# Minimap2onGPU/mm2-gb

Hardware: AMD Instinct MI355X
Metric: chaining anchor-pairs/s (higher is better)
Workload: dtype int32+f32

## Files before the change

include/mm2gb_chain.h:

```cpp
#ifndef MM2GB_CHAIN_H
#define MM2GB_CHAIN_H

#include <stddef.h>
#include <stdint.h>

#ifdef __cplusplus
extern "C" {
#endif

#define MM2GB_VERSION "0.1-mi355x"

typedef struct { uint64_t x, y; } mm2gb_anchor_t;

typedef struct {
	int max_iter, max_dist_x, max_dist_y, max_skip, bw, min_cnt, min_score, is_cdna, n_seg;
	float chn_pen_gap, chn_pen_skip;
} mm2gb_misc_t;

typedef struct {
	int     num_streams;
	int     min_n;
	int64_t long_seg_buffer_size;
	int64_t max_total_n;
	int     max_read;
// ... 24 lines not shown
void mm2gb_config_defaults(mm2gb_config_t *cfg);
int  mm2gb_config_parse(const char *json_text, mm2gb_config_t *cfg);
int  mm2gb_config_load(const char *path, mm2gb_config_t *cfg);

int  mm2gb_device_count(void);
int  mm2gb_device_numa_node(int device);
int  mm2gb_pin_thread_to_device(int device);
int  mm2gb_numa_cpus_for_bdf(const char *bdf, const char *sysfs_root_dir, int32_t *node_out, int32_t *cpus, int32_t max_cpus);
mm2gb_engine_t *mm2gb_engine_create(const mm2gb_config_t *cfg, const mm2gb_misc_t *misc, int device);
void mm2gb_engine_destroy(mm2gb_engine_t *eng);
int  mm2gb_engine_set_misc(mm2gb_engine_t *eng, const mm2gb_misc_t *misc);
int  mm2gb_engine_set_chain_skip(mm2gb_engine_t *eng, int keep);
int  mm2gb_engine_last_score_form(const mm2gb_engine_t *eng);
int  mm2gb_engine_last_score_mode(mm2gb_engine_t *eng);
int  mm2gb_engine_band_groups(const mm2gb_engine_t *eng, int64_t *out);
int  mm2gb_engine_band_shape(const mm2gb_engine_t *eng, int *out6);
int  mm2gb_engine_skip_stats(mm2gb_engine_t *eng, int64_t *out6);
int  mm2gb_engine_device(const mm2gb_engine_t *eng);
int  mm2gb_engine_cu_count(const mm2gb_engine_t *eng);
void mm2gb_engine_gang_counts(const mm2gb_engine_t *eng, int64_t *chunks, int64_t *workgroups);
int  mm2gb_has_gang_build(void);
int  mm2gb_engine_reserve(mm2gb_engine_t *eng, int64_t n_anchors, int64_t n_reads);

int mm2gb_score_host(mm2gb_engine_t *eng, int64_t n_reads, const int64_t *offsets, const mm2gb_anchor_t *anchors,
                     int32_t *f, int32_t *p, mm2gb_stats_t *stats);
int mm2gb_score_device(mm2gb_engine_t *eng, int64_t n_reads, const int64_t *d_offsets, const mm2gb_anchor_t *d_anchors,
                       int64_t n_anchors, int32_t *d_f, int32_t *d_p);
int mm2gb_engine_sync(mm2gb_engine_t *eng);
int mm2gb_engine_stats(mm2gb_engine_t *eng, mm2gb_stats_t *stats);
void *mm2gb_engine_stream(mm2gb_engine_t *eng);
// ... 443 lines not shown
```

mm2-gb_amd/__init__.py:

```python
import ctypes as C
import os

import numpy as np

_HERE = os.path.dirname(os.path.abspath(__file__))
LIB_PATH = os.environ.get("MM2GB_LIB_PATH") or os.path.join(_HERE, "libmm2gb_chain.so")
INT32_MAX = 2**31 - 1


class Misc(C.Structure):
    _fields_ = [("max_iter", C.c_int), ("max_dist_x", C.c_int), ("max_dist_y", C.c_int), ("max_skip", C.c_int),
                ("bw", C.c_int), ("min_cnt", C.c_int), ("min_score", C.c_int), ("is_cdna", C.c_int), ("n_seg", C.c_int),
                ("chn_pen_gap", C.c_float), ("chn_pen_skip", C.c_float)]


class _RangeCfg(C.Structure):
    _fields_ = [("blockdim", C.c_int), ("cut_check_anchors", C.c_int), ("anchor_per_block", C.c_int)]


class _ScoreCfg(C.Structure):
    _fields_ = [("micro_batch", C.c_int), ("mid_blockdim", C.c_int), ("short_griddim", C.c_int), ("long_griddim", C.c_int),
                ("mid_griddim", C.c_int), ("long_seg_cutoff", C.c_int), ("mid_seg_cutoff", C.c_int)]


# ... 264 lines not shown

    def last_score_form(self):
        return int(lib().mm2gb_engine_last_score_form(self._h))

    def last_score_mode(self):
        m = int(lib().mm2gb_engine_last_score_mode(self._h))
        if m < 0:
            raise Mm2gbError(lib().mm2gb_last_error().decode())
        return m

    def band_groups(self):
        out = (C.c_int64 * 2)()
        _check(lib().mm2gb_engine_band_groups(self._h, out))
        return int(out[0]), int(out[1])

    def band_shape(self):
        L = lib()
        L.mm2gb_engine_band_shape.argtypes = [C.c_void_p, C.POINTER(C.c_int)]
        out = (C.c_int * 6)()
        _check(L.mm2gb_engine_band_shape(self._h, out))
        return dict(zip(("slab", "lag_wave", "lag_team4", "lag_team8", "lag_wg", "min_window"), (int(v) for v in out)))

    def cu_count(self):
        L = lib()
        L.mm2gb_engine_cu_count.argtypes = [C.c_void_p]
        return int(L.mm2gb_engine_cu_count(self._h))

    def skip_stats(self):
        L = lib()
        L.mm2gb_engine_skip_stats.argtypes = [C.c_void_p, C.c_void_p]
# ... 1552 lines not shown
```

mm2-gb_amd/csrc/chain_dev.h:

```cpp
#pragma once
#include <hip/hip_runtime.h>
#include <stdint.h>

namespace mm2gb {

struct DevParams {
	int   max_dist_x, max_dist_y, bw, max_iter, n_seg, is_cdna;
	int   dq_lim;
	int   lut_last;
	int   lut_base;
	int   lut_clamp;
	int   free_sweep;
	int   band_slab;
	int   band_lag_wave;
	int   band_lag_team4;
	int   band_lag_team8;
	int   band_lag_wg;
	int   band_min_window;
	float gap, skip;
};
constexpr int BAND_LAG_WAVE = 0, BAND_LAG_TEAM4 = 256, BAND_LAG_TEAM8 = 512, BAND_LAG_WG = 512;
constexpr int BAND_MIN_WINDOW = 256;

enum : unsigned { FLAG_ANY_SEGID = 1u,
                  FLAG_NO_LUT = 2u };

constexpr int LUT_LDS_TOTAL = 31 * 2560;
constexpr int LUT_ENTRIES   = 5120;
constexpr int LUT_LDS_BASE  = LUT_LDS_TOTAL - LUT_ENTRIES * 4;
constexpr int LUT_BIAS      = (1 << 30) + (1 << 16);

constexpr int PLAN_BLOCK = 1024;
#ifndef MM2GB_PLAN_THREADS
#define MM2GB_PLAN_THREADS 256
#endif
constexpr int PLAN_THREADS = MM2GB_PLAN_THREADS;
constexpr int COST_PER_ANCHOR = 16;
// ... 37 lines not shown
	int64_t  *chunk_pp;
	int32_t  *chunk_kk, *chunk_blk;
	int64_t  *tile_sums, *tile_base;
	int32_t  *bins;
	int32_t  *order;
	int32_t  *long_list;
	int32_t  *mid_list;
	int32_t  *counters;
	int64_t  *totals;
	unsigned *flags;
	const int32_t *lut;
	int64_t  *dbg;
	GangSlot *gang_slots;
};
enum { CNT_NCHUNK = 0, CNT_CURSOR = 1, CNT_NLONG = 2, CNT_LCURSOR = 3, CNT_NTRACK = 4, CNT_NCLAMP = 5, CNT_NMID = 6, CNT_MCURSOR = 7,
       CNT_NGANG = 12,
       CNT_GANG_STRIPS = 13,
       CNT_GANG_WGS = 14,
       CNT_BAND_WAVE = 16,
       CNT_BAND_TEAM = 17,
       CNT_WORDS = 18 };

struct LaunchCfg {
	int score_grid;
	int host_mode;
	int ring_slots;
	int big_team;
	int whole_wg_pct;
	int team4_all;
	int team4_share_pct;
	int gang_max;
	int gang_pct;
	int gang_pairs;
	int64_t long_min_cost;
	int     long_min_window;
	int     wide_window;
};

void launch_window(const DevBatch &b, const DevParams &P, hipStream_t s);
void launch_plan(const DevBatch &b, const LaunchCfg &cfg, hipStream_t s);
void launch_score(const DevBatch &b, const DevParams &P, const LaunchCfg &cfg, hipStream_t s);
constexpr int SKIP_STAT_WORDS = 6;
void launch_skip_fill(const DevBatch &b, const DevParams &P, int max_skip, int32_t *mark, unsigned long long *stats, int n_cu, hipStream_t s);
void launch_build_lut(int *d_lut, const DevParams &P, hipStream_t s);
size_t score_lds_bytes(const DevParams &P, int host_mode, int ring_slots);
int  score_set_lds_limit(size_t bytes);
enum { SCORE_MODE_LUT = 0, SCORE_MODE_FAST = 1, SCORE_MODE_GENERAL = 2 };

}
```

mm2-gb_amd/csrc/chain_kernels.hip:

```cpp
#include <hip/hip_runtime.h>
#include <stdint.h>
#include <limits.h>
#include <algorithm>
#include "chain_dev.h"
#include "wave_scan.h"

namespace mm2gb {

#define WAVE 64

__device__ __forceinline__ int lane_id() { return threadIdx.x & (WAVE - 1); }
__device__ __forceinline__ int bcast(int v, int src_lane) { return __builtin_amdgcn_readlane(v, src_lane); }
__device__ __forceinline__ int first_lane(int v) { return __builtin_amdgcn_readfirstlane(v); }
__device__ __forceinline__ int wave_max_i32_dpp(int v)
{
	v = max(v, __builtin_amdgcn_update_dpp(INT_MIN, v, 0x111, 0xf, 0xf, false));
	v = max(v, __builtin_amdgcn_update_dpp(INT_MIN, v, 0x112, 0xf, 0xf, false));
	v = max(v, __builtin_amdgcn_update_dpp(INT_MIN, v, 0x114, 0xf, 0xf, false));
	v = max(v, __builtin_amdgcn_update_dpp(INT_MIN, v, 0x118, 0xf, 0xf, false));
	v = max(v, __builtin_amdgcn_update_dpp(INT_MIN, v, 0x142, 0xa, 0xf, false));
	v = max(v, __builtin_amdgcn_update_dpp(INT_MIN, v, 0x143, 0xc, 0xf, false));
	return __builtin_amdgcn_readlane(v, WAVE - 1);
}
__device__ __forceinline__ int prev_lane(int v) { return __builtin_amdgcn_update_dpp(v, v, 0x138, 0xf, 0xf, false); }
__device__ __forceinline__ int a_x(const DevBatch &b, int i) { return ((const int*)b.raw)[(size_t)i * 4]; }
__device__ __forceinline__ int a_y(const DevBatch &b, int i) { return ((const int*)b.raw)[(size_t)i * 4 + 2]; }
// ... 219 lines not shown
		b.blk_firstcut[blk] = blk_cut;
		b.blk_pairs[blk] = (int64_t)my_pairs;
		b.blk_clamped[blk] = my_clamp;
	}
}

constexpr int PLANNER_THREADS = 1024;
constexpr int N_SMALL_TEAMS_PLAN = 4;
#ifndef MM2GB_COST_BINS_PER_OCTAVE
#define MM2GB_COST_BINS_PER_OCTAVE 16
#endif
constexpr int COST_SUB = MM2GB_COST_BINS_PER_OCTAVE;
constexpr int COST_SUB_LOG = COST_SUB == 16 ? 4 : COST_SUB == 8 ? 3 : 2;
constexpr int COST_BINS = 64 * COST_SUB;
static_assert(COST_BINS <= PLAN_COST_BINS, "the engine allocates PLAN_COST_BINS bins per list");
enum { LIST_WAVE = 0, LIST_BIG = 1, LIST_TEAM4 = 2, N_LISTS = 3 };

__device__ __forceinline__ int cost_bin(int64_t c)
{
	if (c <= 0) return 0;
	const int msb = 63 - __clzll(c);
	const int frac = msb >= COST_SUB_LOG ? (int)((c >> (msb - COST_SUB_LOG)) & (COST_SUB - 1)) : 0;
	return min(COST_BINS - 1, msb * COST_SUB + frac);
}

template <typename T>
__device__ T block_exclusive_scan(T v, T *s_tmp , T *total)
{
	T inc = v;
	for (int off = 1; off < WAVE; off <<= 1) {
		T o = __shfl_up(inc, off);
// ... 69 lines not shown
	for (int k = threadIdx.x; k < N_LISTS * COST_BINS; k += blockDim.x) (&s_hist[0][0])[k] = 0;
	__syncthreads();
	const int n_chunks = b.counters[CNT_NCHUNK];
	int n_track = 0;
	long long big_cost = 0;
	for (int64_t c = (int64_t)blockIdx.x * blockDim.x + threadIdx.x; c < n_chunks; c += (int64_t)gridDim.x * blockDim.x) {
		const bool last = c + 1 >= n_chunks;
		const int start = b.chunk_start[c], end = last ? (int)b.n : b.chunk_start[c + 1];
		const long long pp_next = last ? b.totals[0] : b.chunk_pp[c + 1];
		const long long kk_next = last ? b.totals[1] : (long long)b.chunk_kk[c + 1] + b.blk_clamped[b.chunk_blk[c + 1]];
		const bool track = kk_next - b.chunk_kk[c] > 0;
		const long long cost = (pp_next - b.chunk_pp[c]) + (long long)(end - start) * COST_PER_ANCHOR;
		const long long len = end - start;
		const bool heavy = cfg.ring_slots > 0 && cost >= cfg.long_min_cost && len * cfg.long_min_window <= cost;
		int list = LIST_WAVE;
		if (heavy) {
			const int blk0 = b.chunk_blk[c], blk_end = last ? (int)b.n_blocks : b.chunk_blk[c + 1];
			int wmax = b.blk_wmax[2 * blk0 + 1];
			for (int k = blk0 + 1; k < blk_end; ++k) wmax = max(wmax, b.blk_wmax[2 * k]);
			if (!last) wmax = max(wmax, b.blk_wmax[2 * blk_end]);
			const int need_slots = (wmax + WAVE - 1) / WAVE + 1;
			const int big_slots = cfg.ring_slots / (16 / cfg.big_team), small_slots = cfg.ring_slots / 4;
			const bool lut_build = cfg.host_mode == SCORE_MODE_LUT && !(b.flags[0] & (FLAG_ANY_SEGID | FLAG_NO_LUT));
			const bool small_share = lut_build && (cfg.team4_all || (cfg.team4_share_pct > 0 &&
			                         cost * 100 * cfg.score_grid * N_SMALL_TEAMS_PLAN <= (long long)cfg.team4_share_pct * b.totals[0]));
			if (len * cfg.wide_window > cost && need_slots <= small_slots) list = LIST_TEAM4;
			else if (need_slots <= big_slots) list = small_share ? LIST_TEAM4 : LIST_BIG;
		}
		b.chunk_end[c] = end;
		b.chunk_cost[c] = cost;
		b.chunk_track[c] = (uint8_t)((track ? 1 : 0) | (list << 1));
		n_track += track;
		if (list == LIST_BIG) big_cost += cost;
		atomicAdd(&s_hist[list][cost_bin(cost)], 1);
	}
	__syncthreads();
	for (int k = threadIdx.x; k < N_LISTS * COST_BINS; k += blockDim.x) {
		const int v = (&s_hist[0][0])[k];
		if (v) atomicAdd(&b.bins[k], v);
	}
	for (int off = WAVE / 2; off > 0; off >>= 1) { n_track += __shfl_xor(n_track, off); big_cost += __shfl_xor(big_cost, off); }
	if (lane_id() == 0 && n_track) atomicAdd(&b.counters[CNT_NTRACK], n_track);
	if (lane_id() == 0 && big_cost) atomicAdd((unsigned long long*)&b.totals[2], (unsigned long long)big_cost);
}

__global__ __launch_bounds__(64) void plan_bins(DevBatch b)
{
	if (threadIdx.x < N_LISTS) {
		int acc = 0;
		int *bins = b.bins + threadIdx.x * COST_BINS;
		for (int k = COST_BINS - 1; k >= 0; --k) { const int v = bins[k]; bins[k] = acc; acc += v; }
		if (threadIdx.x == LIST_BIG) b.counters[CNT_NLONG] = acc;
		if (threadIdx.x == LIST_TEAM4) b.counters[CNT_NMID] = acc;
	}
	if (threadIdx.x == 0) { b.counters[CNT_CURSOR] = 0; b.counters[CNT_LCURSOR] = 0; b.counters[CNT_MCURSOR] = 0; }
}

__global__ __launch_bounds__(256) void plan_scatter(DevBatch b)
{
	__shared__ int s_cnt[N_LISTS * COST_BINS], s_base[N_LISTS * COST_BINS];
	const int n_chunks = b.counters[CNT_NCHUNK];
	for (int64_t c0 = (int64_t)blockIdx.x * blockDim.x; c0 < n_chunks; c0 += (int64_t)gridDim.x * blockDim.x) {
		for (int k = threadIdx.x; k < N_LISTS * COST_BINS; k += blockDim.x) s_cnt[k] = 0;
		__syncthreads();
		const int64_t c = c0 + threadIdx.x;
		int key = -1, rank = 0;
		if (c < n_chunks) {
			key = ((b.chunk_track[c] >> 1) & 3) * COST_BINS + cost_bin(b.chunk_cost[c]);
			rank = atomicAdd(&s_cnt[key], 1);
		}
		__syncthreads();
		for (int k = threadIdx.x; k < N_LISTS * COST_BINS; k += blockDim.x) if (s_cnt[k]) s_base[k] = atomicAdd(&b.bins[k], s_cnt[k]);
		__syncthreads();
		if (key >= 0) {
			int *dst = key >= LIST_TEAM4 * COST_BINS ? b.mid_list : key >= LIST_BIG * COST_BINS ? b.long_list : b.order;
			dst[s_base[key] + rank] = (int)c;
		}
		__syncthreads();
	}
}

__global__ __launch_bounds__(256) void plan_gangs(DevBatch b, LaunchCfg cfg)
{
	__shared__ int s_want[256], s_pos[256], s_first[256];
	const int n_long = b.counters[CNT_NLONG];
	const int t = threadIdx.x;
	int want = 0, ci = -1;
	if (t < n_long && cfg.gang_max >= 2 && !(b.flags[0] & (FLAG_ANY_SEGID | FLAG_NO_LUT))) {
		ci = b.long_list[t];
		const long long cost = b.chunk_cost[ci], total = b.totals[0] + (long long)b.n * COST_PER_ANCHOR;
// ... 556 lines not shown
		plain_steps(tl, need & (0xffffull << (16 * q)), bestv);
		if (q < 3) on_quarter(q, bestv);
	}
}

__device__ __forceinline__ bool pair_score_uniform(const DevParams &P, int xi, int yi, int xj, int yj, int tagj, int &sc_out)
{
	const int dq = yi - yj, dr = xi - xj, span = tagj & 0xff;
	const int dg = dr < dq ? dr : dq;
	const int diff = dr - dq;
	const int dd = diff < 0 ? -diff : diff;
	sc_out = (span < dg ? span : dg) - gap_penalty(dd, 0, P);
	return (unsigned)(dq - 1) < (unsigned)P.dq_lim && dr != 0 && dd <= P.bw;
}

template <bool TRACK, typename FOld>
__device__ __forceinline__ void in_tile_lut(const DevBatch &b, const Target &T, int i0, int n_here, const DevParams &P, int4 *stage,
                                            int &best, int &arg, Keep &keep, FOld f_old, const Progress &prog = Progress())
{
	const int lane = lane_id(), i = i0 + lane;
	__builtin_amdgcn_s_setprio(MM2GB_INTILE_PRIO);
	stage[lane] = make_int4(128 - LUT_BIAS, (T.q - 1) * 4, (int)((unsigned)T.x << 2), (int)((unsigned)T.y << 2));
	__builtin_amdgcn_wave_barrier();
	TileLut tl;
	tl.tx4 = (int)(((unsigned)T.x - 1u) << 2); tl.ty4 = (int)(((unsigned)T.y - 1u) << 2);
	tl.lo = T.live ? (T.st > i0 ? T.st - i0 : 0) : WAVE;
	tl.lim4 = (unsigned)P.dq_lim << 2; tl.base = (unsigned)P.lut_base; tl.last_at = tl.base + ((unsigned)P.lut_last << 2);
	tl.stage = stage;
	const int x_prev = prev_lane(T.x);
	tl.edges = __ballot(T.live && (T.st > i0 || (lane > 0 && T.x == x_prev))) != 0;
	tl.kind = P.lut_clamp ? ROWS_CLAMPED : (P.free_sweep && __ballot(T.live && T.st > i0) == 0 &&
	          (unsigned)(bcast(T.x, WAVE - 1) - first_lane(T.x)) <= (unsigned)min(P.dq_lim - P.bw, 1 << 22)) ? ROWS_FREE : ROWS_CHECKED;
	int bestv = (best << 7) - (arg < 0 ? 1 : 0);
	if (!TRACK) {
		if (prog.ring_slot) plain_steps_by_quarters(tl, __ballot(T.live && T.st < i) >> 1, bestv, [&](int q, int bv) { prog.publish(q, bv); });
// ... 284 lines not shown
	if (i0 + WAVE <= t.lo_b) return;
	stage_block_lut(b, i0, f_a, q_a, stage);
	const int eq_lo = equal_x_run_start(b, cs, i0 + WAVE, first_lane(t.B.x));
	const bool no_check = i0 >= t.hi_b && i0 + WAVE <= eq_lo;
	const bool span_ab = P.free_sweep && (unsigned)(t.x_last - t.x_first) <= (unsigned)(P.dq_lim - P.bw);
	sweep_staged_lut(t.B, i0, t.lo_b > i0 ? t.lo_b - i0 : 0, no_check, no_check && span_ab, stage, P, t.best_b, t.arg_b);
	__builtin_amdgcn_wave_barrier();
}

__device__ __forceinline__ int wave_min_i32(int v) { return -wave_max_i32_dpp(-v); }

typedef const int __attribute__((address_space(1))) *glb_i32_cptr;
typedef int __attribute__((address_space(1))) *glb_i32_ptr;
typedef unsigned short __attribute__((address_space(1))) *glb_u16_ptr;
typedef int4 __attribute__((address_space(3))) *lds_i32x4_ptr;
__device__ __forceinline__ int lane_by_count() { return (int)__builtin_amdgcn_mbcnt_hi(~0u, __builtin_amdgcn_mbcnt_lo(~0u, 0u)); }
struct BandParams { int bw, dq_lim, lut_base, free_sweep, band_slab; };
template <class T> __device__ __forceinline__ T uniform_glb(T p)
{
	const unsigned long long v = (unsigned long long)(uintptr_t)p;
	return (T)(uintptr_t)(((unsigned long long)(unsigned)first_lane((int)(v >> 32)) << 32) | (unsigned)first_lane((int)v));
}
__device__ __forceinline__ int r_x(glb_i32_cptr raw, int i) { return raw[(size_t)i * 4]; }
__device__ __forceinline__ int r_y(glb_i32_cptr raw, int i) { return raw[(size_t)i * 4 + 2]; }
__device__ __forceinline__ int r_span(glb_i32_cptr raw, int i) { return (int)((unsigned)raw[(size_t)i * 4 + 3] & 0xffu); }

__device__ __forceinline__ void sweep_block_lut_band(int t_st, int tx4, int ty4, int idx, const int4 *stage, const DevParams &P, int &bestv)
{
	constexpr int G = 4;
	const unsigned base = (unsigned)P.lut_base, lim4 = (unsigned)P.dq_lim << 2;
	int pos = 0x7fffffff;
// ... 293 lines not shown
		}
		if (t.n_b == 0) break;
		sweep_a_into_b(b, t, cs, i0, f_a, TA.q, stage, P);
		const Target TB = load_target(b, i0 + WAVE, ce, TRACK);
		if (in_band && t.lo_b < jl) band_merge(b, i0 + WAVE, t.n_b, t.best_b, t.arg_b);
		in_tile<MODE_LUT, TRACK>(b, TB, i0 + WAVE, t.n_b, P, lut, stage, t.best_b, t.arg_b, keep, f_old);
		if (TB.live) {
			const int i = i0 + WAVE + lane;
			b.f[i] = t.arg_b < 0 ? TB.q : t.best_b;
			b.p[i] = t.arg_b < 0 ? 0 : i - t.arg_b;
		}
	}
	if (band_groups > 0 && lane == 0) atomicAdd(&b.counters[CNT_BAND_WAVE], band_groups);
}

struct CoopShared { int done; int keep[6]; int chunk; int bar_count; int bar_gen; int part; int band; };
#define MM2GB_AGENT __HIP_MEMORY_SCOPE_AGENT
__device__ __forceinline__ int  gload(const int *p) { return __hip_atomic_load(p, __ATOMIC_RELAXED, MM2GB_AGENT); }
__device__ __forceinline__ void gstore(int *p, int v) { __hip_atomic_store(p, v, __ATOMIC_RELAXED, MM2GB_AGENT); }
__device__ __forceinline__ void drain_stores() { asm volatile("s_waitcnt vmcnt(0)" ::: "memory"); }
constexpr int SMALL_TEAM = 4, N_SMALL_TEAMS = SCORE_THREADS / WAVE / SMALL_TEAM;
constexpr int N_TEAM_RECORDS = N_SMALL_TEAMS + 3;
constexpr int TAB_INTS = 12;

__device__ __forceinline__ void team_barrier(CoopShared *sh, int team_size)
{
	__builtin_amdgcn_fence(__ATOMIC_RELEASE, "workgroup");
	if (lane_id() == 0) {
		const int gen = __hip_atomic_load(&sh->bar_gen, __ATOMIC_RELAXED, __HIP_MEMORY_SCOPE_WORKGROUP);
		if (__hip_atomic_fetch_add(&sh->bar_count, 1, __ATOMIC_ACQ_REL, __HIP_MEMORY_SCOPE_WORKGROUP) == team_size - 1) {
// ... 424 lines not shown
	if (ring_slots > 0) {
		int first = -1;
		for (int phase = 0; phase < 3; ++phase) {
			const bool whole = phase == 0, small = phase == 2;
			if (whole && !(big_team < SCORE_THREADS / WAVE && whole_wg_pct > 0)) continue;
			const long long share = whole ? max(1ll, (long long)(b.totals[2] / gridDim.x * whole_wg_pct / 100)) : 0;
			CoopShared *records = small ? teams : whole ? teams + N_SMALL_TEAMS + 2 : teams + N_SMALL_TEAMS;
			const int got = team_phase<MODE, GANG>(b, P, lut, stage, ring, ring_slots, records, small ? b.mid_list : b.long_list, small ? n_mid : n_long,
			                                 small ? CNT_MCURSOR : CNT_LCURSOR, wave, small ? SMALL_TEAM : whole ? SCORE_THREADS / WAVE : big_team,
			                                 whole || small ? -1 : first, share);
			if (whole) first = got;
			if (phase == 1 && b.dbg && lane_id() == 0) atomicMax((unsigned long long*)&b.dbg[blockIdx.x * 4 + 1], (unsigned long long)__builtin_amdgcn_s_memrealtime());
		}
	}
	if (b.dbg && lane_id() == 0) atomicMax((unsigned long long*)&b.dbg[blockIdx.x * 4 + 2], (unsigned long long)__builtin_amdgcn_s_memrealtime());
	const int n_chunks = b.counters[CNT_NCHUNK] - n_long - n_mid;
	while (true) {
		int c = 0;
		if (lane_id() == 0) c = atomicAdd(&b.counters[CNT_CURSOR], 1);
		c = first_lane(c);
		if (c >= n_chunks) break;
		const int ci = first_lane(b.order[c]);
		const int cs = first_lane(b.chunk_start[ci]), ce = first_lane(b.chunk_end[ci]);
		if (MODE == MODE_LUT) {
			const bool band_on = band_chunk(b, P, ci, cs, ce);
			if (b.chunk_track[ci] & 1) run_chunk_pairs<true>(b, P, lut, stage, cs, ce, band_on);
			else run_chunk_pairs<false>(b, P, lut, stage, cs, ce, band_on);
		} else {
			if (b.chunk_track[ci] & 1) run_chunk<MODE, true>(b, P, lut, stage, cs, ce);
			else run_chunk<MODE, false>(b, P, lut, stage, cs, ce);
		}
	}
	if (b.dbg && lane_id() == 0) atomicMax((unsigned long long*)&b.dbg[blockIdx.x * 4 + 3], (unsigned long long)__builtin_amdgcn_s_memrealtime());
}

void launch_window(const DevBatch &b, const DevParams &P, hipStream_t s)
{
	if (b.n <= 0) return;
	hipLaunchKernelGGL(k_block_reads, dim3((unsigned)((b.n_blocks + 255) / 256)), dim3(256), 0, s, b);
	hipLaunchKernelGGL(k_window, dim3((unsigned)b.n_blocks), dim3(PLAN_THREADS), 0, s, b, P);
}

void launch_plan(const DevBatch &b, const LaunchCfg &cfg, hipStream_t s)
{
	const int n_tiles = (int)((b.n_blocks + PLANNER_THREADS - 1) / PLANNER_THREADS);
	const int chunk_grid = (int)std::min<int64_t>(1024, (b.n_blocks + 255) / 256);
	(void)hipMemsetAsync(b.bins, 0, N_LISTS * COST_BINS * sizeof(int), s);
// ... 183 lines not shown
```

mm2-gb_amd/csrc/engine.h:

```cpp
#pragma once
#include <hip/hip_runtime.h>
#include <stdint.h>
#include <functional>
#include <string>
#include <vector>
#include "../../include/mm2gb_chain.h"
#include "chain_dev.h"
#include "post_dev.h"
#include "seed_dev.h"

namespace mm2gb {

void set_error(const std::string &msg);
int  index_on_device(const mm2gb_index_t *ix, int device, DevIndexView *out);
void retire_device_buffer(void *ptr, size_t bytes);
int  fail(const std::string &msg);

#define MM2GB_HIP(call)                                                                                        \
	do {                                                                                                       \
		hipError_t e_ = (call);                                                                                \
		if (e_ != hipSuccess)                                                                                  \
			return ::mm2gb::fail(std::string(#call) + ": " + hipGetErrorString(e_));                           \
	} while (0)

// ... 78 lines not shown
	hipEvent_t post0 = nullptr, post1 = nullptr;
	hipEvent_t post_fork = nullptr, post_join = nullptr;
	IoSet io[2];
	uint64_t io_seq = 0;
	PinnedBuf h_slice_off;
	std::vector<hipEvent_t> slice_in;
	PinnedBuf h_res_f, h_res_p;
	char    *h_small = nullptr;
	int32_t *h_counters = nullptr;
	int64_t *h_totals = nullptr;
	BatchSlot slots[MAX_SLOTS];
	int n_slots = 0;

	mm2gb_stats_t last = {};
	bool misc_valid = false, coop_disabled = false, debug_phases = false, one_compute_stream = false;
	int64_t team4_min_n = 0;
	int64_t gang_max_n = 0;
	int64_t last_gang_chunks = 0, last_gang_wgs = 0;
	bool rmq_tiles_last = false;
	std::function<void(const int32_t*)> rmq_tied_ready;
	hipEvent_t rmq_fill_done = nullptr;
	int  rmq_team_reads = 0;
	bool rmq_abandon_tied = false;
	bool rmq_calibrate = false;
	int  rmq_kernel = 0;
	bool lds_contract_ok = false;
	int64_t dual_stream_max_n = 16 * 1000 * 1000;
	bool chain_skip = false;
	int64_t last_band_groups[2] = { 0, 0 };
	int  last_score_form = 0;
	int  last_score_set = 0, last_score_host_mode = 0;
	bool skip_stats = false;
	int  last_skip_set = 0;

	int  init(const mm2gb_config_t *cfg, const mm2gb_misc_t *misc, int device);
	void shutdown();
	int  set_misc(const mm2gb_misc_t *m);
	int  configure_score();
	int  reserve(int64_t n_anchors, int64_t n_reads, int set = 0);
	int  begin_call();
	int  enqueue_host(int64_t n_reads, const int64_t *h_offsets, const mm2gb_anchor_t *h_anchors, int64_t n, int32_t *h_f, int32_t *h_p, bool want_stats = true);
	int  enqueue(int64_t n_reads, const int64_t *d_offsets, const mm2gb_anchor_t *d_anchors, int64_t n, int32_t *d_f, int32_t *d_p, bool want_stats = true, int set = 0);
	int  score_host(int64_t n_reads, const int64_t *offsets, const mm2gb_anchor_t *anchors, int32_t *f, int32_t *p,
// ... 43 lines not shown
```

mm2-gb_amd/csrc/engine.hip:

```cpp
#include <atomic>
#include <hip/hip_runtime.h>
#include <sys/mman.h>
#include <mutex>
#include <algorithm>
#include <chrono>
#include <cstdio>
#include <cstdlib>
#include <cstring>
#include <vector>
#include <string>
#include "engine.h"
#include "est_err.h"
#include "host_chain.h"
#include "seed_heap.h"

namespace mm2gb {

static thread_local std::string g_err;
void set_error(const std::string &msg) { g_err = msg; }
int fail(const std::string &msg) { g_err = msg; return -1; }
const char *last_error_cstr() { return g_err.c_str(); }

static size_t grown(size_t need, size_t have)
{
// ... 328 lines not shown
	hipDeviceProp_t prop;
	MM2GB_HIP(hipGetDeviceProperties(&prop, device));
	n_cu = prop.multiProcessorCount > 0 ? prop.multiProcessorCount : 256;
	cfg = *c;
	launch.score_grid = cfg.score_kernel.short_griddim > 0 ? std::max(1, cfg.score_kernel.short_griddim / 4) : n_cu * 2;
	launch.long_min_window = 128;
	launch.long_min_cost = (int64_t)std::max(1, cfg.score_kernel.mid_seg_cutoff) * std::max(64, cfg.range_kernel.blockdim) * 1024;
	launch.wide_window = 1024;
	if (const char *v = getenv("MM2GB_LONG_MIN_WINDOW")) launch.long_min_window = std::max(1, atoi(v));
	if (const char *v = getenv("MM2GB_WIDE_WINDOW")) launch.wide_window = std::max(1, atoi(v));
	if (const char *v = getenv("MM2GB_LONG_MIN_COST")) launch.long_min_cost = std::max<int64_t>(1, atoll(v));
	launch.team4_all = 0; launch.team4_share_pct = 60; team4_min_n = 250000000;
	if (const char *v = getenv("MM2GB_TEAM4_ALL")) launch.team4_all = atoi(v) != 0;
	if (const char *v = getenv("MM2GB_TEAM4_SHARE_PCT")) launch.team4_share_pct = std::max(0, atoi(v));
	if (const char *v = getenv("MM2GB_TEAM4_MIN_ANCHORS")) team4_min_n = std::max<int64_t>(0, atoll(v));
	if (const char *v = getenv("MM2GB_DEBUG_PHASES")) debug_phases = *v && *v != '0';
	if (const char *v = getenv("MM2GB_CHAIN_SKIP")) chain_skip = strcmp(v, "keep") == 0;
	{ const char *v = getenv("MM2GB_SKIP_STATS"); skip_stats = v && *v && *v != '0'; }
	launch.gang_max = 8; launch.gang_pct = 150; gang_max_n = 150000000;
	if (const char *v = getenv("MM2GB_GANG_MAX")) launch.gang_max = std::max(0, std::min(64, atoi(v)));
	if (const char *v = getenv("MM2GB_GANG_PCT")) launch.gang_pct = std::max(1, atoi(v));
	launch.gang_pairs = 0;
	if (const char *v = getenv("MM2GB_GANG_PAIRS")) launch.gang_pairs = *v && *v != '0';
	if (const char *v = getenv("MM2GB_GANG_MAX_ANCHORS")) gang_max_n = std::max<int64_t>(0, atoll(v));
	if (debug_phases && dbg.ensure((size_t)launch.score_grid * 32)) return -1;
	const char *env = getenv("MM2GB_NO_COOP");
	coop_disabled = env && *env && *env != '0';
	{
		const int before = dev >= 0 && dev < MAX_COUNTED_DEVICES ? g_engines_on_device[dev].fetch_add(1) : 0;
		counted_on_device = dev >= 0 && dev < MAX_COUNTED_DEVICES;
// ... 77 lines not shown
int Engine::reserve(int64_t n, int64_t n_reads, int set)
{
	MM2GB_HIP(hipSetDevice(device));
	if (n >= ((int64_t)1 << 31) - 2 * PLAN_BLOCK) return fail("mm2gb: a micro-batch is limited to 2^31 anchors (got " + std::to_string(n) + ")");
	WorkSet &w = work[set];
	if (n > w.cap_n || n_reads > w.cap_reads) {
		MM2GB_HIP(hipStreamSynchronize(w.stream));
		const int64_t nn = std::max<int64_t>(std::max(n, w.cap_n), 1024);
		const int64_t nb = (nn + PLAN_BLOCK - 1) / PLAN_BLOCK + 1;
		const int64_t had_reads = w.cap_reads;
		w.cap_n = w.cap_blocks = w.cap_reads = 0;
		if (w.st.ensure(nn * 4)) return -1;
		if (w.blk_firstcut.ensure(nb * 4) || w.blk_pairs.ensure(nb * 8) || w.blk_clamped.ensure(nb * 4) || w.blk_wmax.ensure(nb * 8) || w.blk_read.ensure(nb * 4)) return -1;
		if (w.chunk_start.ensure(nb * 4) || w.chunk_end.ensure(nb * 4) || w.chunk_cost.ensure(nb * 8) || w.chunk_track.ensure(nb) ||
		    w.order.ensure(nb * 4) || w.long_list.ensure(nb * 4) || w.mid_list.ensure(nb * 4) || w.chunk_pp.ensure(nb * 8) || w.chunk_kk.ensure(nb * 4) || w.chunk_blk.ensure(nb * 4) ||
		    w.tile_sums.ensure((nb / 1024 + 2) * 24) || w.tile_base.ensure((nb / 1024 + 2) * 24) || w.bins.ensure(3 * PLAN_COST_BINS * 4)) return -1;
		w.cap_n = nn; w.cap_blocks = nb; w.cap_reads = std::max(had_reads, n_reads);
	}
	return 0;
}

int Engine::begin_call()
{
	if (n_slots > 0 && sync()) return -1;
	n_slots = 0;
	last = mm2gb_stats_t();
	last_gang_chunks = last_gang_wgs = 0;
	last_band_groups[0] = last_band_groups[1] = 0;
	return 0;
}

int Engine::enqueue(int64_t n_reads, const int64_t *d_offsets, const mm2gb_anchor_t *d_anchors, int64_t n, int32_t *d_f, int32_t *d_p, bool want_stats, int set)
{
	if (n < 0 || n_reads < 0) return fail("mm2gb: negative batch size");
	if (want_stats && n_slots >= MAX_SLOTS && sync()) return -1;
	if (reserve(n, n_reads, set)) return -1;
	WorkSet &w = work[set];
	hipStream_t stream = w.stream;
	DevBuf &st = w.st, &blk_firstcut = w.blk_firstcut, &blk_pairs = w.blk_pairs, &blk_clamped = w.blk_clamped, &blk_wmax = w.blk_wmax,
	       &blk_read = w.blk_read, &chunk_start = w.chunk_start, &chunk_end = w.chunk_end, &chunk_cost = w.chunk_cost, &chunk_track = w.chunk_track, &order = w.order,
	       &long_list = w.long_list, &mid_list = w.mid_list, &chunk_pp = w.chunk_pp, &chunk_kk = w.chunk_kk, &chunk_blk = w.chunk_blk, &tile_sums = w.tile_sums,
	       &tile_base = w.tile_base, &bins = w.bins, &counters = w.counters, &totals = w.totals, &flags = w.flags;
	const int slot = want_stats ? n_slots++ : 0;
// ... 9 lines not shown
	b.chunk_start = (int32_t*)chunk_start.ptr; b.chunk_end = (int32_t*)chunk_end.ptr; b.chunk_cost = (int64_t*)chunk_cost.ptr;
	b.chunk_track = (uint8_t*)chunk_track.ptr; b.order = (int32_t*)order.ptr; b.long_list = (int32_t*)long_list.ptr; b.mid_list = (int32_t*)mid_list.ptr;
	b.chunk_pp = (int64_t*)chunk_pp.ptr; b.chunk_kk = (int32_t*)chunk_kk.ptr; b.chunk_blk = (int32_t*)chunk_blk.ptr;
	b.tile_sums = (int64_t*)tile_sums.ptr; b.tile_base = (int64_t*)tile_base.ptr; b.bins = (int32_t*)bins.ptr;
	b.counters = (int32_t*)counters.ptr; b.totals = (int64_t*)totals.ptr; b.flags = (unsigned*)flags.ptr;
	b.lut = (const int32_t*)lut.ptr;
	b.dbg = debug_phases ? (int64_t*)dbg.ptr : nullptr;
	if (debug_phases) MM2GB_HIP(hipMemsetAsync(dbg.ptr, 0, (size_t)launch.score_grid * 32, stream));
	LaunchCfg cfg_now = launch;
	if (n < team4_min_n) cfg_now.team4_share_pct = 0;
	b.gang_slots = nullptr;
	if (launch.gang_max >= 2 && launch.host_mode == SCORE_MODE_LUT && launch.ring_slots > 0 && n > 0 && n <= gang_max_n) {
		if (w.gang_slots.ensure((size_t)GANG_MAX_CHUNKS * sizeof(GangSlot))) return -1;
		b.gang_slots = (GangSlot*)w.gang_slots.ptr;
	}

	MM2GB_HIP(hipMemsetAsync(counters.ptr, 0, CNT_WORDS * sizeof(int32_t), stream));
	MM2GB_HIP(hipMemsetAsync(totals.ptr, 0, 4 * sizeof(int64_t), stream));
	MM2GB_HIP(hipMemsetAsync(flags.ptr, 0, 4 * sizeof(unsigned), stream));
	if (want_stats) MM2GB_HIP(hipEventRecord(bs.prep0, stream));
	if (n > 0) {
		launch_window(b, params, stream);
		launch_plan(b, cfg_now, stream);
	}
	if (want_stats) MM2GB_HIP(hipEventRecord(bs.prep1, stream));
	const bool walk = chain_skip && misc.max_skip < misc.max_iter;
	last_score_form = walk ? 1 : 0;
	last_score_set = set; last_score_host_mode = launch.host_mode;
	if (n > 0 && walk) {
		if (w.skip_mark.ensure((size_t)n * sizeof(int32_t))) return -1;
// ... 880 lines not shown
				for (int w = 0; w < launch.score_grid; ++w) if (h[4 * w]) for (int k = 0; k < 8; ++k) busy[k] += h[4 * w + 3] - t0 > e3 * k / 8;
				fprintf(stderr, "[mm2gb phases] workgroups still at work after 0/8 ... 7/8 of the kernel's time: %d %d %d %d %d %d %d %d\n", busy[0], busy[1], busy[2], busy[3], busy[4], busy[5], busy[6], busy[7]);
			}
		}
	}
	for (int k = 0; k < n_slots; ++k) {
		const int32_t *c = h_counters + (size_t)k * CNT_WORDS;
		last.n_pairs += h_totals[(size_t)k * 2];
		last.n_chunks += c[CNT_NCHUNK];
		last.n_long_chunks += c[CNT_NLONG];
		last.n_mid_chunks += c[CNT_NMID];
		last.n_tracked_chunks += c[CNT_NTRACK];
		last.n_clamped_blocks += c[CNT_NCLAMP];
		last_gang_chunks += c[CNT_NGANG]; last_gang_wgs += c[CNT_GANG_WGS];
		last_band_groups[0] += c[CNT_BAND_WAVE]; last_band_groups[1] += c[CNT_BAND_TEAM];
		float ms = 0;
		if (hipEventElapsedTime(&ms, slots[k].prep0, slots[k].prep1) == hipSuccess) last.ms_prep += ms;
		if (hipEventElapsedTime(&ms, slots[k].prep1, slots[k].score1) == hipSuccess) last.ms_score += ms;
	}
	if (n_slots > 0) last.ms_total = last.ms_prep + last.ms_score;
	n_slots = 0;
	return 0;
}

int Engine::score_host(int64_t n_reads, const int64_t *offsets, const mm2gb_anchor_t *anchors, int32_t *f, int32_t *p,
                       const std::function<void(int64_t, int64_t)> *slice_done)
{
	const int64_t base = offsets[0], n = offsets[n_reads] - base;
	for (int64_t r = 0; r < n_reads; ++r) if (offsets[r + 1] < offsets[r]) return fail("mm2gb_score_host: offsets must be non-decreasing");
	if (n > 0 && (!anchors || !f || !p)) return fail("mm2gb_score_host: null buffer");
// ... 100 lines not shown
int mm2gb_engine_last_score_mode(mm2gb_engine_t *eng)
{
	if (!eng) return -1;
	Engine &e = eng->e;
	if (!e.work[e.last_score_set].flags.ptr) return fail("mm2gb_engine_last_score_mode: engine not initialised");
	if (e.sync()) return -1;
	unsigned fl = 0;
	MM2GB_HIP(hipMemcpy(&fl, e.work[e.last_score_set].flags.ptr, sizeof fl, hipMemcpyDeviceToHost));
	const int host_mode = e.last_score_host_mode;
	return (fl & FLAG_ANY_SEGID) ? SCORE_MODE_GENERAL : (host_mode == SCORE_MODE_LUT && (fl & FLAG_NO_LUT)) ? SCORE_MODE_FAST : host_mode;
}
int mm2gb_engine_band_groups(const mm2gb_engine_t *eng, int64_t *out)
{
	if (!eng || !out) return fail("mm2gb_engine_band_groups: null argument");
	out[0] = eng->e.last_band_groups[0]; out[1] = eng->e.last_band_groups[1];
	return 0;
}
int mm2gb_engine_band_shape(const mm2gb_engine_t *eng, int *out)
{
	if (!eng || !out) return fail("mm2gb_engine_band_shape: null argument");
	const DevParams &P = eng->e.params;
	out[0] = P.band_slab; out[1] = P.band_lag_wave; out[2] = P.band_lag_team4; out[3] = P.band_lag_team8; out[4] = P.band_lag_wg; out[5] = P.band_min_window;
	return 0;
}
int mm2gb_engine_skip_stats(mm2gb_engine_t *eng, int64_t *out)
{
	if (!eng || !out) return fail("mm2gb_engine_skip_stats: null argument");
	Engine &e = eng->e;
	if (!e.skip_stats || !e.work[e.last_skip_set].skip_stats.ptr) return fail("mm2gb_engine_skip_stats: no counters (MM2GB_SKIP_STATS=1 when the engine is made, then a call that ran the walk)");
	if (e.sync()) return -1;
// ... 327 lines not shown
```

Before: 7503 billion.

## Add sparse-chunk list scored by a lean noinline wave path

The planner adds a fourth list for non-tracked, non-heavy chunks whose widest window is at most 63 anchors. These chunks go into the tail of the order array. In LUT mode without gang scheduling, a separate noinline routine scores them by claiming groups of eight. It uses a simplified per-tile sweep that carries the previous tile's last anchor forward instead of running the general chunk path. The path is only enabled when a batch has at least 250M anchors (tunable by environment variable), which adds a counter, a stats getter and one more bins list in exchange for cheaper scoring of short-window chunks.

```diff
diff --git a/include/mm2gb_chain.h b/include/mm2gb_chain.h
--- a/include/mm2gb_chain.h
+++ b/include/mm2gb_chain.h
@@ -62,6 +62,7 @@
 int  mm2gb_engine_last_score_form(const mm2gb_engine_t *eng);
 int  mm2gb_engine_last_score_mode(mm2gb_engine_t *eng);
 int  mm2gb_engine_band_groups(const mm2gb_engine_t *eng, int64_t *out);
+int  mm2gb_engine_sparse_chunks(const mm2gb_engine_t *eng, int64_t *scored);
 int  mm2gb_engine_band_shape(const mm2gb_engine_t *eng, int *out6);
 int  mm2gb_engine_skip_stats(mm2gb_engine_t *eng, int64_t *out6);
 int  mm2gb_engine_device(const mm2gb_engine_t *eng);
diff --git a/mm2-gb_amd/__init__.py b/mm2-gb_amd/__init__.py
--- a/mm2-gb_amd/__init__.py
+++ b/mm2-gb_amd/__init__.py
@@ -302,6 +302,13 @@
         _check(lib().mm2gb_engine_band_groups(self._h, out))
         return int(out[0]), int(out[1])
 
+    def sparse_chunks(self):
+        L = lib()
+        L.mm2gb_engine_sparse_chunks.argtypes = [C.c_void_p, C.POINTER(C.c_int64)]
+        n = C.c_int64()
+        _check(L.mm2gb_engine_sparse_chunks(self._h, C.byref(n)))
+        return int(n.value)
+
     def band_shape(self):
         L = lib()
         L.mm2gb_engine_band_shape.argtypes = [C.c_void_p, C.POINTER(C.c_int)]
diff --git a/mm2-gb_amd/csrc/chain_dev.h b/mm2-gb_amd/csrc/chain_dev.h
--- a/mm2-gb_amd/csrc/chain_dev.h
+++ b/mm2-gb_amd/csrc/chain_dev.h
@@ -21,6 +21,8 @@
 };
 constexpr int BAND_LAG_WAVE = 0, BAND_LAG_TEAM4 = 256, BAND_LAG_TEAM8 = 512, BAND_LAG_WG = 512;
 constexpr int BAND_MIN_WINDOW = 256;
+constexpr int SPARSE_WINDOW_LIMIT = 63, SPARSE_MAX_WINDOW = 63;
+static_assert(SPARSE_WINDOW_LIMIT < 64 && SPARSE_WINDOW_LIMIT < BAND_MIN_WINDOW, "a sparse chunk never takes the band pass");
 
 enum : unsigned { FLAG_ANY_SEGID = 1u,
                   FLAG_NO_LUT = 2u };
@@ -88,12 +90,17 @@
 	GangSlot *gang_slots;
 };
 enum { CNT_NCHUNK = 0, CNT_CURSOR = 1, CNT_NLONG = 2, CNT_LCURSOR = 3, CNT_NTRACK = 4, CNT_NCLAMP = 5, CNT_NMID = 6, CNT_MCURSOR = 7,
+       CNT_NWAVE = 8,
+       CNT_NSPARSE = 9,
+       CNT_SCURSOR = 10,
+       CNT_SPARSE_DONE = 11,
        CNT_NGANG = 12,
        CNT_GANG_STRIPS = 13,
        CNT_GANG_WGS = 14,
        CNT_BAND_WAVE = 16,
        CNT_BAND_TEAM = 17,
        CNT_WORDS = 18 };
+constexpr int PLAN_LISTS = 4;
 
 struct LaunchCfg {
 	int score_grid;
@@ -109,6 +116,7 @@
 	int64_t long_min_cost;
 	int     long_min_window;
 	int     wide_window;
+	int     sparse_max_window;
 };
 
 void launch_window(const DevBatch &b, const DevParams &P, hipStream_t s);
diff --git a/mm2-gb_amd/csrc/chain_kernels.hip b/mm2-gb_amd/csrc/chain_kernels.hip
--- a/mm2-gb_amd/csrc/chain_kernels.hip
+++ b/mm2-gb_amd/csrc/chain_kernels.hip
@@ -10,6 +10,7 @@
 #define WAVE 64
 
 __device__ __forceinline__ int lane_id() { return threadIdx.x & (WAVE - 1); }
+__device__ __forceinline__ int lane_by_count() { return (int)__builtin_amdgcn_mbcnt_hi(~0u, __builtin_amdgcn_mbcnt_lo(~0u, 0u)); }
 __device__ __forceinline__ int bcast(int v, int src_lane) { return __builtin_amdgcn_readlane(v, src_lane); }
 __device__ __forceinline__ int first_lane(int v) { return __builtin_amdgcn_readfirstlane(v); }
 __device__ __forceinline__ int wave_max_i32_dpp(int v)
@@ -259,7 +260,8 @@
 constexpr int COST_SUB_LOG = COST_SUB == 16 ? 4 : COST_SUB == 8 ? 3 : 2;
 constexpr int COST_BINS = 64 * COST_SUB;
 static_assert(COST_BINS <= PLAN_COST_BINS, "the engine allocates PLAN_COST_BINS bins per list");
-enum { LIST_WAVE = 0, LIST_BIG = 1, LIST_TEAM4 = 2, N_LISTS = 3 };
+enum { LIST_WAVE = 0, LIST_BIG = 1, LIST_TEAM4 = 2, LIST_SPARSE = 3, N_LISTS = 4 };
+static_assert(N_LISTS == PLAN_LISTS, "the engine allocates PLAN_LISTS lists of bins");
 
 __device__ __forceinline__ int cost_bin(int64_t c)
 {
@@ -359,11 +361,15 @@
 		const long long len = end - start;
 		const bool heavy = cfg.ring_slots > 0 && cost >= cfg.long_min_cost && len * cfg.long_min_window <= cost;
 		int list = LIST_WAVE;
-		if (heavy) {
+		auto widest_window = [&]() {
 			const int blk0 = b.chunk_blk[c], blk_end = last ? (int)b.n_blocks : b.chunk_blk[c + 1];
 			int wmax = b.blk_wmax[2 * blk0 + 1];
 			for (int k = blk0 + 1; k < blk_end; ++k) wmax = max(wmax, b.blk_wmax[2 * k]);
 			if (!last) wmax = max(wmax, b.blk_wmax[2 * blk_end]);
+			return wmax;
+		};
+		if (heavy) {
+			const int wmax = widest_window();
 			const int need_slots = (wmax + WAVE - 1) / WAVE + 1;
 			const int big_slots = cfg.ring_slots / (16 / cfg.big_team), small_slots = cfg.ring_slots / 4;
 			const bool lut_build = cfg.host_mode == SCORE_MODE_LUT && !(b.flags[0] & (FLAG_ANY_SEGID | FLAG_NO_LUT));
@@ -371,7 +377,7 @@
 			                         cost * 100 * cfg.score_grid * N_SMALL_TEAMS_PLAN <= (long long)cfg.team4_share_pct * b.totals[0]));
 			if (len * cfg.wide_window > cost && need_slots <= small_slots) list = LIST_TEAM4;
 			else if (need_slots <= big_slots) list = small_share ? LIST_TEAM4 : LIST_BIG;
-		}
+		} else if (!track && cfg.sparse_max_window > 0 && widest_window() <= min(cfg.sparse_max_window, SPARSE_WINDOW_LIMIT)) list = LIST_SPARSE;
 		b.chunk_end[c] = end;
 		b.chunk_cost[c] = cost;
 		b.chunk_track[c] = (uint8_t)((track ? 1 : 0) | (list << 1));
@@ -397,8 +403,10 @@
 		for (int k = COST_BINS - 1; k >= 0; --k) { const int v = bins[k]; bins[k] = acc; acc += v; }
 		if (threadIdx.x == LIST_BIG) b.counters[CNT_NLONG] = acc;
 		if (threadIdx.x == LIST_TEAM4) b.counters[CNT_NMID] = acc;
-	}
-	if (threadIdx.x == 0) { b.counters[CNT_CURSOR] = 0; b.counters[CNT_LCURSOR] = 0; b.counters[CNT_MCURSOR] = 0; }
+		if (threadIdx.x == LIST_WAVE) b.counters[CNT_NWAVE] = acc;
+		if (threadIdx.x == LIST_SPARSE) b.counters[CNT_NSPARSE] = acc;
+	}
+	if (threadIdx.x == 0) { b.counters[CNT_CURSOR] = 0; b.counters[CNT_LCURSOR] = 0; b.counters[CNT_MCURSOR] = 0; b.counters[CNT_SCURSOR] = 0; }
 }
 
 __global__ __launch_bounds__(256) void plan_scatter(DevBatch b)
@@ -418,7 +426,8 @@
 		for (int k = threadIdx.x; k < N_LISTS * COST_BINS; k += blockDim.x) if (s_cnt[k]) s_base[k] = atomicAdd(&b.bins[k], s_cnt[k]);
 		__syncthreads();
 		if (key >= 0) {
-			int *dst = key >= LIST_TEAM4 * COST_BINS ? b.mid_list : key >= LIST_BIG * COST_BINS ? b.long_list : b.order;
+			const int list = key / COST_BINS;
+			int *dst = list == LIST_TEAM4 ? b.mid_list : list == LIST_BIG ? b.long_list : list == LIST_SPARSE ? b.order + b.counters[CNT_NWAVE] : b.order;
 			dst[s_base[key] + rank] = (int)c;
 		}
 		__syncthreads();
@@ -1005,11 +1014,11 @@
 	return (unsigned)(dq - 1) < (unsigned)P.dq_lim && dr != 0 && dd <= P.bw;
 }
 
-template <bool TRACK, typename FOld>
+template <bool TRACK, typename FOld, bool BY_COUNT = false>
 __device__ __forceinline__ void in_tile_lut(const DevBatch &b, const Target &T, int i0, int n_here, const DevParams &P, int4 *stage,
                                             int &best, int &arg, Keep &keep, FOld f_old, const Progress &prog = Progress())
 {
-	const int lane = lane_id(), i = i0 + lane;
+	const int lane = BY_COUNT ? lane_by_count() : lane_id(), i = i0 + lane;
 	__builtin_amdgcn_s_setprio(MM2GB_INTILE_PRIO);
 	stage[lane] = make_int4(128 - LUT_BIAS, (T.q - 1) * 4, (int)((unsigned)T.x << 2), (int)((unsigned)T.y << 2));
 	__builtin_amdgcn_wave_barrier();
@@ -1324,7 +1333,6 @@
 typedef int __attribute__((address_space(1))) *glb_i32_ptr;
 typedef unsigned short __attribute__((address_space(1))) *glb_u16_ptr;
 typedef int4 __attribute__((address_space(3))) *lds_i32x4_ptr;
-__device__ __forceinline__ int lane_by_count() { return (int)__builtin_amdgcn_mbcnt_hi(~0u, __builtin_amdgcn_mbcnt_lo(~0u, 0u)); }
 struct BandParams { int bw, dq_lim, lut_base, free_sweep, band_slab; };
 template <class T> __device__ __forceinline__ T uniform_glb(T p)
 {
@@ -1648,6 +1656,77 @@
 	if (band_groups > 0 && lane == 0) atomicAdd(&b.counters[CNT_BAND_WAVE], band_groups);
 }
 
+typedef unsigned u32x4_t __attribute__((ext_vector_type(4)));
+typedef const u32x4_t __attribute__((address_space(1))) *glb_u32x4_cptr;
+struct SparseParams { int bw, dq_lim, lut_base, lut_last, lut_clamp, free_sweep; };
+__device__ __noinline__ void sparse_chunk(const glb_u32x4_cptr raw_, const glb_i32_cptr st_, const glb_i32_ptr f_, const glb_i32_ptr p_,
+                                          const SparseParams sp, const lds_i32x4_ptr stage_, const int cs_, const int ce_)
+{
+	const glb_u32x4_cptr raw = uniform_glb(raw_);
+	const glb_i32_cptr st = uniform_glb(st_);
+	const glb_i32_ptr f = uniform_glb(f_), p = uniform_glb(p_);
+	DevParams P = {};
+	P.bw = first_lane(sp.bw); P.dq_lim = first_lane(sp.dq_lim); P.lut_base = first_lane(sp.lut_base); P.lut_last = first_lane(sp.lut_last);
+	P.lut_clamp = first_lane(sp.lut_clamp); P.free_sweep = first_lane(sp.free_sweep);
+	int4 *stage = (int4*)(lds_i32x4_ptr)(uintptr_t)(unsigned)first_lane((int)(unsigned)(uintptr_t)stage_);
+	const int cs = first_lane(cs_), ce = first_lane(ce_);
+	const int lane = lane_by_count();
+	const DevBatch none = {};
+	Keep keep; keep.idx = -1; keep.x = keep.hi = keep.y = keep.tag = keep.f = 0;
+	int px = 0, py = 0, pq = 0, pf = 0;
+	for (int i0 = cs; i0 < ce; i0 += WAVE) {
+		const int i = i0 + lane, n_here = min(WAVE, ce - i0);
+		Target T;
+		T.live = i < ce;
+		const int il = T.live ? i : ce - 1;
+		const u32x4_t a = raw[il];
+		T.x = (int)a.x; T.y = (int)a.z; T.tag = tag_of(a.w); T.hi = 0;
+		T.st = T.live ? st[il] : INT_MAX;
+		T.q = T.tag & 0xff; T.seg = T.tag >> 8;
+		int best = T.q + 1, arg = -1;
+		const int tile_lo = first_lane(T.st);
+		if (tile_lo < i0) {
+			const int jb = i0 - WAVE;
+			stage_block_lut_at(lane, px, py, pf, pq, stage);
+			const TileXY xy = { T.x, T.y, T.st };
+			sweep_staged_lut(xy, jb, max(tile_lo - jb, 0), false, false, stage, P, best, arg);
+			__builtin_amdgcn_wave_barrier();
+		}
+		if ((__ballot(T.live && T.st < i) >> 1) != 0ull)
+			in_tile_lut<false, int (*)(int), true>(none, T, i0, n_here, P, stage, best, arg, keep, nullptr);
+		const int fi = arg < 0 ? T.q : best;
+		if (T.live) {
+			f[i] = fi;
+			p[i] = arg < 0 ? 0 : i - arg;
+		}
+		px = T.x; py = T.y; pq = T.q; pf = fi;
+	}
+}
+__device__ __forceinline__ void sparse_run(const DevBatch &b, const DevParams &P, int4 *stage, const int ci)
+{
+	const SparseParams sp = { P.bw, P.dq_lim, P.lut_base, P.lut_last, P.lut_clamp, P.free_sweep };
+	sparse_chunk((glb_u32x4_cptr)(const u32x4_t*)b.raw, (glb_i32_cptr)b.st, (glb_i32_ptr)b.f, (glb_i32_ptr)b.p, sp, (lds_i32x4_ptr)stage,
+	             first_lane(b.chunk_start[ci]), first_lane(b.chunk_end[ci]));
+}
+constexpr int SPARSE_CLAIM = 8;
+__device__ __forceinline__ int sparse_take(const DevBatch &b, const DevParams &P, int4 *stage, const int n_sparse)
+{
+	const int32_t *list = b.order + first_lane(b.counters[CNT_NWAVE]);
+	int taken = 0;
+	int seen = 0;
+	while (seen < n_sparse) {
+		int c = 0;
+		if (lane_id() == 0) c = atomicAdd(&b.counters[CNT_SCURSOR], SPARSE_CLAIM);
+		c = first_lane(c);
+		seen = c + SPARSE_CLAIM;
+		if (c < n_sparse) {
+			const int c_end = min(c + SPARSE_CLAIM, n_sparse);
+			for (int k = c; k < c_end; ++k) sparse_run(b, P, stage, first_lane(list[k]));
+			taken += c_end - c;
+		}
+	}
+	return taken;
+}
 struct CoopShared { int done; int keep[6]; int chunk; int bar_count; int bar_gen; int part; int band; };
 #define MM2GB_AGENT __HIP_MEMORY_SCOPE_AGENT
 __device__ __forceinline__ int  gload(const int *p) { return __hip_atomic_load(p, __ATOMIC_RELAXED, MM2GB_AGENT); }
@@ -2102,12 +2181,17 @@
 		}
 	}
 	if (b.dbg && lane_id() == 0) atomicMax((unsigned long long*)&b.dbg[blockIdx.x * 4 + 2], (unsigned long long)__builtin_amdgcn_s_memrealtime());
-	const int n_chunks = b.counters[CNT_NCHUNK] - n_long - n_mid;
+	const bool lean = MODE == MODE_LUT && !GANG;
+	const int n_wave = GANG ? b.counters[CNT_NCHUNK] - n_long - n_mid : first_lane(b.counters[CNT_NWAVE]);
+	const int n_sparse = GANG ? 0 : first_lane(b.counters[CNT_NSPARSE]);
+	const int n_chunks = lean ? n_wave : n_wave + n_sparse;
+	int n_tail = 0;
 	while (true) {
 		int c = 0;
 		if (lane_id() == 0) c = atomicAdd(&b.counters[CNT_CURSOR], 1);
 		c = first_lane(c);
 		if (c >= n_chunks) break;
+		if (!GANG) n_tail += c >= n_wave;
 		const int ci = first_lane(b.order[c]);
 		const int cs = first_lane(b.chunk_start[ci]), ce = first_lane(b.chunk_end[ci]);
 		if (MODE == MODE_LUT) {
@@ -2119,6 +2203,8 @@
 			else run_chunk<MODE, false>(b, P, lut, stage, cs, ce);
 		}
 	}
+	if (lean && n_sparse > 0) n_tail = sparse_take(b, P, stage, n_sparse);
+	if (n_tail > 0 && lane_id() == 0) atomicAdd(&b.counters[CNT_SPARSE_DONE], n_tail);
 	if (b.dbg && lane_id() == 0) atomicMax((unsigned long long*)&b.dbg[blockIdx.x * 4 + 3], (unsigned long long)__builtin_amdgcn_s_memrealtime());
 }
 
diff --git a/mm2-gb_amd/csrc/engine.h b/mm2-gb_amd/csrc/engine.h
--- a/mm2-gb_amd/csrc/engine.h
+++ b/mm2-gb_amd/csrc/engine.h
@@ -116,6 +116,7 @@
 
 	mm2gb_stats_t last = {};
 	bool misc_valid = false, coop_disabled = false, debug_phases = false, one_compute_stream = false;
+	int64_t sparse_min_n = 0;
 	int64_t team4_min_n = 0;
 	int64_t gang_max_n = 0;
 	int64_t last_gang_chunks = 0, last_gang_wgs = 0;
@@ -129,6 +130,7 @@
 	bool lds_contract_ok = false;
 	int64_t dual_stream_max_n = 16 * 1000 * 1000;
 	bool chain_skip = false;
+	int64_t last_sparse_chunks = 0;
 	int64_t last_band_groups[2] = { 0, 0 };
 	int  last_score_form = 0;
 	int  last_score_set = 0, last_score_host_mode = 0;
diff --git a/mm2-gb_amd/csrc/engine.hip b/mm2-gb_amd/csrc/engine.hip
--- a/mm2-gb_amd/csrc/engine.hip
+++ b/mm2-gb_amd/csrc/engine.hip
@@ -366,6 +366,9 @@
 	if (const char *v = getenv("MM2GB_TEAM4_ALL")) launch.team4_all = atoi(v) != 0;
 	if (const char *v = getenv("MM2GB_TEAM4_SHARE_PCT")) launch.team4_share_pct = std::max(0, atoi(v));
 	if (const char *v = getenv("MM2GB_TEAM4_MIN_ANCHORS")) team4_min_n = std::max<int64_t>(0, atoll(v));
+	launch.sparse_max_window = SPARSE_MAX_WINDOW; sparse_min_n = 250000000;
+	if (const char *v = getenv("MM2GB_SPARSE_MIN_ANCHORS")) sparse_min_n = std::max<int64_t>(0, atoll(v));
+	if (const char *v = getenv("MM2GB_SPARSE_MAX_WINDOW")) launch.sparse_max_window = std::max(0, std::min(SPARSE_WINDOW_LIMIT, atoi(v)));
 	if (const char *v = getenv("MM2GB_DEBUG_PHASES")) debug_phases = *v && *v != '0';
 	if (const char *v = getenv("MM2GB_CHAIN_SKIP")) chain_skip = strcmp(v, "keep") == 0;
 	{ const char *v = getenv("MM2GB_SKIP_STATS"); skip_stats = v && *v && *v != '0'; }
@@ -473,7 +476,7 @@
 		if (w.blk_firstcut.ensure(nb * 4) || w.blk_pairs.ensure(nb * 8) || w.blk_clamped.ensure(nb * 4) || w.blk_wmax.ensure(nb * 8) || w.blk_read.ensure(nb * 4)) return -1;
 		if (w.chunk_start.ensure(nb * 4) || w.chunk_end.ensure(nb * 4) || w.chunk_cost.ensure(nb * 8) || w.chunk_track.ensure(nb) ||
 		    w.order.ensure(nb * 4) || w.long_list.ensure(nb * 4) || w.mid_list.ensure(nb * 4) || w.chunk_pp.ensure(nb * 8) || w.chunk_kk.ensure(nb * 4) || w.chunk_blk.ensure(nb * 4) ||
-		    w.tile_sums.ensure((nb / 1024 + 2) * 24) || w.tile_base.ensure((nb / 1024 + 2) * 24) || w.bins.ensure(3 * PLAN_COST_BINS * 4)) return -1;
+		    w.tile_sums.ensure((nb / 1024 + 2) * 24) || w.tile_base.ensure((nb / 1024 + 2) * 24) || w.bins.ensure(PLAN_LISTS * PLAN_COST_BINS * 4)) return -1;
 		w.cap_n = nn; w.cap_blocks = nb; w.cap_reads = std::max(had_reads, n_reads);
 	}
 	return 0;
@@ -486,6 +489,7 @@
 	last = mm2gb_stats_t();
 	last_gang_chunks = last_gang_wgs = 0;
 	last_band_groups[0] = last_band_groups[1] = 0;
+	last_sparse_chunks = 0;
 	return 0;
 }
 
@@ -525,6 +529,7 @@
 		if (w.gang_slots.ensure((size_t)GANG_MAX_CHUNKS * sizeof(GangSlot))) return -1;
 		b.gang_slots = (GangSlot*)w.gang_slots.ptr;
 	}
+	if (n < sparse_min_n || b.gang_slots) cfg_now.sparse_max_window = 0;
 
 	MM2GB_HIP(hipMemsetAsync(counters.ptr, 0, CNT_WORDS * sizeof(int32_t), stream));
 	MM2GB_HIP(hipMemsetAsync(totals.ptr, 0, 4 * sizeof(int64_t), stream));
@@ -1435,6 +1440,7 @@
 		last.n_clamped_blocks += c[CNT_NCLAMP];
 		last_gang_chunks += c[CNT_NGANG]; last_gang_wgs += c[CNT_GANG_WGS];
 		last_band_groups[0] += c[CNT_BAND_WAVE]; last_band_groups[1] += c[CNT_BAND_TEAM];
+		last_sparse_chunks += c[CNT_SPARSE_DONE];
 		float ms = 0;
 		if (hipEventElapsedTime(&ms, slots[k].prep0, slots[k].prep1) == hipSuccess) last.ms_prep += ms;
 		if (hipEventElapsedTime(&ms, slots[k].prep1, slots[k].score1) == hipSuccess) last.ms_score += ms;
@@ -1565,6 +1571,12 @@
 {
 	if (!eng || !out) return fail("mm2gb_engine_band_groups: null argument");
 	out[0] = eng->e.last_band_groups[0]; out[1] = eng->e.last_band_groups[1];
+	return 0;
+}
+int mm2gb_engine_sparse_chunks(const mm2gb_engine_t *eng, int64_t *scored)
+{
+	if (!eng || !scored) return fail("mm2gb_engine_sparse_chunks: null argument");
+	*scored = eng->e.last_sparse_chunks;
 	return 0;
 }
 int mm2gb_engine_band_shape(const mm2gb_engine_t *eng, int *out)
```

After: 7892 billion, median of 6. 5.2% higher.
